# dimalit/ipt

Hardware: AMD Instinct MI355X
Metric: Mpaths/sec at 1024^2, 8-bounce, sample_scenes[0]; achieved HBM GB/s (higher is better)
Workload: dtype f32; 1 GPU; c2: box 1024x1024, 1280 spp, depth_max 8, n_rays 16; width=1024, height=1024, spp=1280, depth_max=8, n_rays=16, tile_rows=0, calls=queued (ipt_render_device_async), one wait, parallelism=tiles1, per_rank=the whole frame's tiles dealt round-robin; 256 x N passes per step (weak)

## Files before the change

ipt_amd/csrc/ipt_kernels.hip:

```cpp
#include <hip/hip_runtime.h>

#include <algorithm>
#include <array>
#include <cmath>
#include <cstdio>
#include <cstdlib>
#include <cstring>
#include <strings.h>
#include <mutex>
#include <string>
#include <thread>
#include <type_traits>
#include <vector>

#include "../../include/ipt_capi.h"
#include "ipt_bvh.h"
#include "ipt_internal.h"
#include "ipt_path.h"
#include "ipt_knobs.h"
#include "ipt_diag.h"

using namespace ipt;

namespace {
// ... 783 lines not shown
        const bool sharded = !(kp.n_shards <= 1 || kp.tile_rows <= 0);
        uint4 r0, r1;
        compact_record(kp, (uint32_t)unit, sharded, r0, r1);
        if (c < kp.total_units) {
            rg[2 * c] = r0;
            rg[2 * c + 1] = r1;
            src[c] = (uint32_t)unit;
        }
    }
}

__global__ void compact_preset_kernel(const unsigned int* __restrict__ blocks, unsigned int nblk,
                                      unsigned long long total_units, unsigned long long* __restrict__ unit_counter,
                                      unsigned long long* __restrict__ ring) {
    if (blockIdx.x != 0 || threadIdx.x != 0) return;
    const unsigned long long n_active = blocks[nblk];
    const unsigned long long start = (total_units - n_active) / kPoolChunk * kPoolChunk;
    *unit_counter = start;
    ring[0] = start;
    ring[1] = n_active;
}

__global__ __launch_bounds__(256) void compact_expand_kernel(const CompactBufs cb, unsigned int nblk,
                                                             unsigned long long total_units) {
    const unsigned long long c = (unsigned long long)blockIdx.x * blockDim.x + threadIdx.x;
    if (c >= total_units || c < total_units - cb.blocks[nblk]) return;
    cb.values[cb.src[c]] = cb.cvalues[c];
}

template <int MAXSUSP, bool COUNT, int LMODE, int GEOM, bool BOXIN, int FIXED>
__global__ __launch_bounds__(block_of(LMODE, GEOM), waves_per_simd(GEOM, LMODE)) void path_kernel(const KParams kp) {
    static_assert(!BOXIN || GEOM == IPT_GEOM_SPHERE_IN_BOX, "BOXIN is the box instances' parameter");
    static_assert(!FIXED || (BOXIN && step_fixed_mode(LMODE)), "FIXED: in-range box instances with a skip-ahead plane");
    static_assert(FIXED >= kFixedPow2 && FIXED <= MAXSUSP, "FIXED = K: K suspended levels");
    constexpr bool kFixed = FIXED != 0;
    constexpr int kK = FIXED > 0 ? FIXED : 0;
    constexpr int kTreeRays = 1 << kK, kTreeMetaShift = kTreeRays > 255 ? 16 : 8;
    constexpr int kRange = GEOM == IPT_GEOM_SPHERE_IN_BOX ? (BOXIN ? kRangeIn : kRangeGeneric) : kRangeRuntime;
    constexpr bool kNearest = box_nearest(GEOM) && kRange != kRangeGeneric;
    constexpr int kBlock = block_of(LMODE, GEOM);
    extern __shared__ float lds[];
    unsigned long long* wslots = reinterpret_cast<unsigned long long*>(lds);
    float* stk = lds + walk_lds_words(LMODE, GEOM);
    constexpr int kFrameStride = frame_stride(LMODE, GEOM);
    float* lfr = stk + MAXSUSP * kStackFields * kBlock;
    LightDev* lights_lds = reinterpret_cast<LightDev*>(lfr + 12 * kFrameStride);
    float* weights_lds = reinterpret_cast<float*>(lights_lds) + kLdsLights * kLightWords;
    float* cdf_lds = weights_lds + (kLdsLights + 1);
    float* gl_lds = reinterpret_cast<float*>(lights_lds) +
                    (LMODE == kLightsLds ? kLdsLights * kLightWords + 2 * (kLdsLights + 1) : 0);
    constexpr bool kGridL = grid_lights(LMODE);
    BvhNode* lnodes_lds = reinterpret_cast<BvhNode*>(gl_lds + global_light_prefix_words(kp.n_lights, kGridL));
    float* cdf_gl = gl_lds + (kGridL ? 0 : kp.n_lights + 1);
    constexpr bool kLaxLds = lax_in_lds(LMODE);
    float4* lax_lds = reinterpret_cast<float4*>(reinterpret_cast<int*>(lnodes_lds) + ((kp.lg_nu * kp.lg_nv + 3) & ~3));
    int* cdf_lo_lds = reinterpret_cast<int*>(cdf_gl + kp.n_lights + 1);
    const int tid = threadIdx.x;
    const int wave = tid >> 6;
    if (tid < 60) lfr[(tid % 12) * kFrameStride + kBlock + tid / 12] = reinterpret_cast<const float*>(kp.wall_frames)[tid];
    if (LMODE == kLightsLds) {
        const float* src = reinterpret_cast<const float*>(kp.lights);
        float* dst = reinterpret_cast<float*>(lights_lds);
        for (int i = tid; i < kp.n_lights * kLightWords; i += kBlock) dst[i] = src[i];
        for (int i = tid; i <= kp.n_lights; i += kBlock) {
            weights_lds[i] = kp.weights[i];
            cdf_lds[i] = kp.cdf[i];
        }
    }
    if (global_lights(LMODE)) {
        const bool int_cdf = kp.cdf_p2;
        for (int i = tid; i <= kp.n_lights; i += kBlock) {
            if (!kGridL) gl_lds[i] = kp.weights[i];
            cdf_gl[i] = int_cdf ? __uint_as_float(cdf_threshold24(kp.cdf[i])) : kp.cdf[i];
        }
        if (kp.cdf_lo)
            for (int i = tid; i < kCdfBuckets; i += kBlock) cdf_lo_lds[i] = kp.cdf_lo[i];
        if (grid_lights(LMODE))
            for (int i = tid; i < kp.lg_nu * kp.lg_nv; i += kBlock) reinterpret_cast<int*>(lnodes_lds)[i] = kp.lgrid[i];
        if (kLaxLds)
            for (int i = tid; i < 3 * kp.n_lights; i += kBlock) lax_lds[i] = kp.lax[i];
        if (LMODE == kLightsGlobal && kp.lnodes_lds) {
            const float4* src = reinterpret_cast<const float4*>(kp.light_nodes);
            float4* dst = reinterpret_cast<float4*>(lnodes_lds);
            for (int i = tid; i < 2 * kp.n_light_nodes; i += kBlock) dst[i] = src[i];
        }
    }
    __syncthreads();
    LightSet<LMODE> LS;
    LS.lds = lights_lds;
    LS.glob = kp.lights;
    LS.wl = global_lights(LMODE) ? gl_lds : weights_lds;
    LS.cl = global_lights(LMODE) ? cdf_gl : cdf_lds;
    LS.wg = kp.weights;
    LS.cg = kp.cdf;
    if (one_light(LMODE)) {
        LS.one = kp.lights[0];
        if (!resumable_geom(GEOM)) {
            vgpr_hold(LS.one.P); vgpr_hold(LS.one.x); vgpr_hold(LS.one.y);
            vgpr_hold(LS.one.n); vgpr_hold(LS.one.inv.c[0]); vgpr_hold(LS.one.inv.c[1]); vgpr_hold(LS.one.inv.c[2]);
        }
        LS.w0 = kp.weights[0];
        LS.c0 = kp.cdf[0];
        LS.c1 = kp.cdf[1];
    }

    auto ltrace = [&](const LightDev& L, vec3 o, vec3 d, vec3* hp, vec3* hn) -> bool {
        if constexpr (LMODE == kLightsOneA10) return light_trace_ax<1, 0, true>(L, o, d, hp, hn);
        else if constexpr (LMODE == kLightsOneA01) return light_trace_ax<0, 1, true>(L, o, d, hp, hn);
        else if constexpr (grid_lights(LMODE) && lattice_a10(LMODE)) return light_trace_ax<1, 0, true>(L, o, d, hp, hn);
        else if constexpr (grid_lights(LMODE)) return light_trace_ax<0, 1, true>(L, o, d, hp, hn);
        else return light_trace<LMODE == kLightsAny>(L, o, d, hp, hn);
    };
    auto lpdf = [&](const LightDev& L, vec3 o, bool h, vec3 hp, vec3 hn) -> float {
        if constexpr (LMODE == kLightsOneA10 || LMODE == kLightsOneA01) return light_pdf_ax<2, true>(L, o, h, hp, hn);
        else if constexpr (grid_lights(LMODE)) return light_pdf_ax<2, true>(L, o, h, hp, hn);
        else return light_pdf(L, o, h, hp, hn);
    };
    auto lsample = [&](const LightDev& L, vec3 o, float a, float b) -> vec3 {
        if constexpr (LMODE == kLightsOneA10) return light_sample_dir_ax<1, 0, true>(L, o, a, b);
        else if constexpr (LMODE == kLightsOneA01) return light_sample_dir_ax<0, 1, true>(L, o, a, b);
        else if constexpr (grid_lights(LMODE) && lattice_a10(LMODE)) return light_sample_dir_ax<1, 0, true>(L, o, a, b);
        else if constexpr (grid_lights(LMODE)) return light_sample_dir_ax<0, 1, true>(L, o, a, b);
        else return light_sample_dir<LMODE == kLightsAny>(L, o, a, b);
    };

    const int lane = tid & 63;
    const uint64_t lanemask_lt = (lane == 0) ? 0ull : (~0ull >> (64 - lane));
    const int nl = one_light(LMODE) ? 1 : kp.n_lights;
    const float w_sdf = kp.weights[nl];
    const unsigned long long per_pass = (unsigned long long)kp.n_cand * (unsigned long long)kp.W;

    __builtin_amdgcn_s_waitcnt(0);

    unsigned long long pool_next = 0, pool_end = 0;

    bool active = true, has_path = false, fresh = false, need_frame = false, need_b = false;
    int pick = -1;
    float u1 = 0.0f, u2 = 0.0f, tr = 0.0f, cs_c = 0.0f, cs_s = 0.0f;
    float pfs = 0.0f, pfc = 0.0f;
    vec3 pto = v3(0, 0, 0);
    bool pfok = false;
    uint32_t unit = 0;
    uint32_t rpass = 0, rpix = 0, k = 0, blk = 0;
    Win8 w;
    vec3 tpos = v3(0, 0, 0);
    int fdepth = -1;
    uint32_t finm = 0;
    constexpr bool kRes = resumable_geom(GEOM);
    constexpr bool kResL = resumable_lights(LMODE, GEOM);
    constexpr bool kBoxHit = !kRes && !kResL && GEOM == IPT_GEOM_SPHERE_IN_BOX && kNearest;
    constexpr bool kFramePf = !(kRes || kResL);
    constexpr bool kSkipAhead = (one_light(LMODE) || grid_lights(LMODE)) && !kResL;
    constexpr bool kPreSkip = kSkipAhead && kFramePf;
    bool tracing = false;
    float xlmix = 0.0f;
    vec3 xro = v3(0, 0, 0), xrd = v3(0, 0, 0), xli_pos = v3(0, 0, 0);
    int xrdepth = 0, xi = 0, xbidx = -1;
    float xli_y = 0.0f;
    bool xis_iter = false, xhas_li = false;
    float xmult = 0.0f, xli_pow = 0.0f, xbest = 0.0f;
    vec3 xtm = v3(0, 0, 0);
    float tres = 0.0f;
    int ti = 0, tdepth = 0, tkind = 0;
    uint32_t c_paths = 0, c_traced = 0, c_surf = 0, c_light = 0, c_exp = 0, c_iter = 0,
             c_lsamp = 0, c_skip = 0, c_sframe = 0, c_ltr = 0, c_drift = 0, c_nodes = 0, c_tests = 0,
             c_lnode = 0, c_ltest = 0;
    IPT_DIAG_STATE

    for (;;) {
        IPT_STAMP_AT(0);
        const bool need = active && !has_path;
        const uint64_t needmask = __ballot(need);
        if (needmask) {
            const int cnt = __popcll(needmask);
            const int rank = __popcll(needmask & lanemask_lt);
            unsigned long long avail = pool_end - pool_next;
            unsigned long long my = 0;
            if ((unsigned long long)cnt > avail) {
                unsigned long long base = 0;
                if (lane == __ffsll((long long)needmask) - 1) {
                    base = atomicAdd(kp.unit_counter, (unsigned long long)kPoolChunk);
                    if (kp.drained && base + kPoolChunk >= kp.total_units)
                        __hip_atomic_store(kp.drained, kp.drain_seq, __ATOMIC_RELAXED, __HIP_MEMORY_SCOPE_SYSTEM);
                }
                base = __shfl(base, __ffsll((long long)needmask) - 1);
                if ((unsigned long long)rank < avail)
                    my = pool_next + rank;
                else
                    my = base + (rank - avail);
                pool_next = base + (cnt - avail);
                pool_end = base + kPoolChunk;
            } else {
                my = pool_next + rank;
                pool_next += cnt;
            }
            if (need) {
                if (my >= kp.total_units) {
                    active = false;
                } else {
                    unit = (uint32_t)my;
                    has_path = true;
                    fresh = true;
                }
            }
        }

        IPT_STAMP_AT(1);
        if (active) { IPT_PHASE(0); }
        auto pop_node = [&]() {
        if (has_path && (kFramePf || !fresh) && !((kRes || kResL) && tracing) && ti >= ((kK > 0 ? kTreeRays : kp.n_rays) >> tdepth)) {
            IPT_PHASE(1);
            const uint32_t m = ~finm & ((1u << tdepth) - 1u);
            const int stop = m ? 31 - (int)__clz(m) : -1;
            constexpr int kLevelWords = kStackFields * kBlock;
            const lds_float* sb = (const lds_float*)(stk + tid);
            auto lvl = [&](int l) { return sb + __umul24((uint32_t)(l < 0 ? 0 : l), (uint32_t)kLevelWords); };
            const lds_float* bs = lvl(stop);
            const float s0 = bs[0 * kBlock], s1 = bs[1 * kBlock], s2 = bs[2 * kBlock];
            const float s3 = bs[3 * kBlock], s4 = bs[4 * kBlock], s5 = bs[5 * kBlock];
            const lds_float* b1 = lvl(tdepth - 1);
            const float r1 = b1[3 * kBlock], m1 = b1[4 * kBlock];
            const lds_float* b2 = lvl(tdepth - 2);
            const float r2 = b2[3 * kBlock], m2 = b2[4 * kBlock];
            uint32_t nr = kK > 0 ? 1u << kK : (uint32_t)kp.n_rays;
            if constexpr (kK == 0) asm volatile("" : "+s"(nr));
            const bool n_pow2 = kFixed || (nr != 0u && (nr & (nr - 1u)) == 0u);
            const uint32_t p2_exp = 96u + (uint32_t)__clz((int)nr);
            float v;
            auto unwind = [&](auto p2) {
                constexpr bool kP2 = decltype(p2)::value;
                const uint32_t sc0 = (p2_exp + (uint32_t)tdepth) << 23;
                auto fin_s = [&](float r, int d, uint32_t sc) {
                    const float q = kP2 ? r * __uint_as_float(sc) : r / (float)(kp.n_rays >> (d < 0 ? 0 : d));
                    return isfinite_(r) ? q : 0.0f;
                };
                v = fin_s(tres, tdepth, sc0);
                const float v1 = fin_s(r1 + (m1 * 1.0f) * v, tdepth - 1, sc0 - (1u << 23));
                v = tdepth - 1 > stop ? v1 : v;
                const float v2 = fin_s(r2 + (m2 * 1.0f) * v, tdepth - 2, sc0 - (2u << 23));
                v = tdepth - 2 > stop ? v2 : v;
                uint32_t sc = sc0 - (3u << 23);
#pragma unroll 1
                for (int l = tdepth - 3; l > stop; --l, sc -= 1u << 23) {
                    const lds_float* b = lvl(l);
                    const float r = b[3 * kBlock] + (b[4 * kBlock] * 1.0f) * v;
                    v = 0.0f;
                    if (isfinite_(r)) v = kP2 ? r * __uint_as_float(sc) : r / (float)(kp.n_rays >> l);
                }
            };
            if constexpr (kFixed)
                unwind(std::true_type{});
            else if (n_pow2)
                unwind(std::true_type{});
            else
                unwind(std::false_type{});
            if (stop >= 0) {
                const int meta = __float_as_int(s5);
                tpos = v3(s0, s1, s2);
                tres = s3 + (s4 * 1.0f) * v;
                tkind = (int)((uint32_t)meta >> (kK > 0 ? kTreeMetaShift : kp.meta_shift));
                ti = (int)__builtin_amdgcn_ubfe((uint32_t)meta, 0u, (uint32_t)(kK > 0 ? kTreeMetaShift : kp.meta_shift));
                need_frame = tkind >= 5 && fdepth != stop;
                tdepth = stop;
                vgpr_hold(tpos);
                vgpr_hold(tdepth);
            } else {
                kp.values[unit] = v >= 0.0f ? v : 0.0f;
                has_path = false;
            }
        }
        };
        if (!kFramePf) pop_node();

        IPT_STAMP_AT(2);
        auto frame_normal = [&]() -> vec3 {
            vec3 nrm;
            if (GEOM == IPT_GEOM_SPHERE_IN_BOX || tkind == 5) {
                nrm = tpos;
            } else {
                const float4 sp = kp.spheres[tkind - 6];
                nrm = tpos - v3(sp.x, sp.y, sp.z);
                if (GEOM == IPT_GEOM_SMALLPT && !((double)sp.w < 100.0)) nrm = -nrm;
            }
            return nrm;
        };
        constexpr bool kFrameInrange = GEOM == IPT_GEOM_SPHERE_IN_BOX;
        const bool fneed = need_frame && has_path && !fresh && !((kRes || kResL) && tracing);
        IPT_STAMP_AT(3);
        const bool iter_lane = has_path && !fresh && !((kRes || kResL) && tracing);
        if constexpr (kRes) {
            pick = -1;
            u1 = u2 = tr = cs_c = cs_s = 0.0f;
        }
        uint32_t gi_a = 0, gi_b = 0;
        bool gcos = false;
        uint32_t pre_w;
        bool pre_ok = false;
        bool pre_ft;
        vec3 lpP = v3(0, 0, 0);
        float lpx = 0.0f, lpy = 0.0f, lpn = 0.0f;
        int lptype = 0;
        auto gathers = [&](bool ran) {
            if constexpr (kRes || kResL) {
                if (ran && gcos) {
                    tr = kp.cos_a[gi_a];
                    float sp, cp;
                    sincosf_small_(two_pi_times_u24(gi_b), &sp, &cp);
                    cs_c = cp;
                    cs_s = sp;
                }
            } else {
                if constexpr (grid_lights(LMODE)) {
                    const int pk = (ran && pick >= 0 && pick < nl) ? pick : 0;
                    const float4 a = kLaxLds ? lax_lds[3 * pk] : kp.lax[3 * pk];
                    lpP = v3(a.x, a.y, kp.lg_pn);
                    lpx = a.z;
                    lpy = a.w;
                    lpn = kp.lg_nn;
                    lptype = 0;
                }
                tr = kp.cos_a[gcos ? gi_a : 0u];
                float sp, cp;
                sincosf_small_(two_pi_times_u24(gi_b), &sp, &cp);
                cs_c = cp;
                cs_s = sp;
            }
        };
        auto prologue = [&]() {
            if ((k >> 2) != blk) {
                w.a0 = w.b0; w.a1 = w.b1; w.a2 = w.b2; w.a3 = w.b3;
                ++blk;
                need_b = true;
            }
            if (need_b) {
                IPT_PHASE(4);
                philox_fill(w.b0, w.b1, w.b2, w.b3, blk + 1, rpass, rpix, kp.key0, kp.key1);
                need_b = false;
            }
            const uint32_t j = kPreSkip ? k - 4u * blk : k & 3u;
            const uint32_t rw = kPreSkip && j >= 4u ? (j & 1u ? w.b1 : w.b0) : sel4(j & 3u, w.a0, w.a1, w.a2, w.a3);
            const float r = u01(rw);
            auto pick_w = [&](uint32_t wd) {
                return (unsigned long long)wd < kp.pk_u0 ? 0 : ((unsigned long long)wd < kp.pk_u1 ? 1 : 2);
            };
            constexpr bool kPickInt = one_light(LMODE);
            auto pick_of = [&](float r) {
                int c = 0;
                if (global_lights(LMODE) && kp.cdf_lo) {
                    c = cdf_lo_lds[(int)(r * 256.0f)];
                    if (kp.cdf_bsearch) {
                        const float f0 = LS.cdf(min(c, nl)), f1 = LS.cdf(min(c + 1, nl)), f2 = LS.cdf(min(c + 2, nl));
                        const int n0 = (c <= nl && !(r < f0)) ? 1 : 0;
                        const int n1 = (c + 1 <= nl && !(r < f1)) ? 1 : 0;
                        const int n2 = (c + 2 <= nl && !(r < f2)) ? 1 : 0;
                        const bool more = n2 != 0;
                        c += n0 + n1 + n2;
                        if (__builtin_expect(__any(more), 0))
                            if (more) while (c <= nl && !(r < LS.cdf(c))) ++c;
                    } else {
                        while (c <= nl && !(r < LS.cdf(c))) ++c;
                    }
                } else if ((global_lights(LMODE) || LMODE == kLightsAny) && kp.cdf_bsearch) {
                    int hi = nl + 1;
                    while (c < hi) {
                        const int mid = (c + hi) >> 1;
                        if (r < LS.cdf(mid)) hi = mid; else c = mid + 1;
                    }
                } else {
                    while (c <= nl && !(r < LS.cdf(c))) ++c;
                }
                return c;
            };
            auto pick_p2w = [&](uint32_t wd) {
                const uint32_t g = wd >> 8;
                const int ce = min((int)(g >> (24 - kp.cdf_p2e)), nl);
                if (kp.cdf_p2 == 2) {
                    return ce < nl ? ce : (g < kp.cdf_end_t ? nl : nl + 1);
                }
                const uint32_t fa = __float_as_uint(LS.cdf(max(ce - 1, 0))), fb = __float_as_uint(LS.cdf(ce));
                int c = (ce >= 1 && g < fa) ? ce - 1 : (g < fb ? ce : ce + 1);
                if (c >= nl) c = g < kp.cdf_end_t ? nl : nl + 1;
                return c;
            };
            constexpr bool kPickIntCdf = global_lights(LMODE);
            auto pick_word = [&](uint32_t wd) {
                if constexpr (kPickInt) return pick_w(wd);
                if constexpr (kPickIntCdf)
                    if (kp.cdf_p2) return pick_p2w(wd);
                return pick_of(u01(wd));
            };
            int c = (kPickInt || kPickIntCdf) ? pick_word(rw) : pick_of(r);
            uint32_t jj = j;
            if constexpr (kSkipAhead) {
                const bool back = (tpos.z - kp.sa_pz) * kp.sa_nz < 0.0f;
                if ((kFixed || kp.sa_on) && c < nl && back && j <= 1u && ti + 1 < ((kK > 0 ? kTreeRays : kp.n_rays) >> tdepth)) {
                    ++ti;
                    if (COUNT) { ++c_iter; ++c_lsamp; ++c_skip; }
                    k += 3;
                    jj = j + 3u;
                    c = pick_word(j == 0u ? w.a3 : w.b0);
                }
            }
            pick = c;
            if (c <= nl) {
                uint32_t r1, r2;
                if constexpr (kPreSkip) {
                    const bool odd = (jj & 1u) != 0u, h0 = jj < 2u, h2 = jj >= 4u;
                    auto sel3 = [&](uint32_t x0, uint32_t x1, uint32_t x2) {
                        const uint32_t t = h0 ? x0 : x1;
                        return h2 ? x2 : t;
                    };
                    const uint32_t e1 = sel3(w.a1, w.a3, w.b1), e2 = sel3(w.a2, w.b0, w.b2);
                    const uint32_t e3 = sel3(w.a3, w.b1, w.b3), e4 = h0 ? w.b0 : w.b2;
                    r1 = odd ? e2 : e1;
                    r2 = odd ? e3 : e2;
                    pre_w = odd ? e4 : e3;
                    pre_ok = jj <= 3u && (kFixed || kp.sa_on);
                    if constexpr (kK > 0 && !COUNT)
                        pre_ft = kPickIntCdf ? (pre_w >> 8) >= kp.cdf_end_t : pick_word(pre_w) > nl;
                } else {
                    const bool hi = kSkipAhead && jj >= 4u;
                    r1 = hi ? w.b1 : sel4(jj & 3u, w.a1, w.a2, w.a3, w.b0);
                    r2 = hi ? w.b2 : sel4(jj & 3u, w.a2, w.a3, w.b0, w.b1);
                }
                u1 = u01(r1);
                u2 = u01(r2);
                if (c == nl) {
                    gi_a = r1 >> 8;
                    gi_b = r2 >> 8;
                    gcos = true;
                }
                k += 3;
            } else {
                k += 1;
            }
        };
        if (iter_lane) {
            IPT_PHASE(3);
            prologue();
        }
        gathers(iter_lane);
        if (fneed) {
            const vec3 nrm = frame_normal();
            IPT_PHASE(5);
            Frame f;
            if (GEOM == IPT_GEOM_SPHERE_IN_BOX) {
                vec3 to;
                float fs = 0.0f, fc = 0.0f;
                if (kFramePf) {
                    if (__builtin_expect(__any(!pfok), 0))
                        if (!pfok) {
                            pto = kFrameInrange ? normalize_inrange_(nrm) : normalize(nrm);
                            frame_sc_lookup(kp.frame_sc, pto, pfs, pfc);
                            keep_alive(pfs);
                            keep_alive(pfc);
                        }
                    to = pto;
                    fs = pfs;
                    fc = pfc;
                    pfok = false;
                } else {
                    to = kFrameInrange ? normalize_inrange_(nrm) : normalize(nrm);
                    frame_sc_lookup(kp.frame_sc, to, fs, fc);
                }
                if (kFrameInrange) {
                    bool ok;
                    f = make_frame_sc_fast(to, fs, fc, ok);
                    if (__builtin_expect(__any(!ok), 0))
                        if (!ok) f = make_frame_sc<kFrameInrange>(to, fs, fc);
                } else {
                    f = make_frame_sc<kFrameInrange>(to, fs, fc);
                }
            } else if (kFrameInrange) {
                f = make_frame<true>(normalize_inrange_(nrm));
            } else {
                const vec3 to = normalize(nrm);
                float fs, fc;
                frame_angle_sc(to, &fs, &fc);
                bool ok;
                f = make_frame_sc_fast(to, fs, fc, ok);
                if (__builtin_expect(__any(!ok), 0))
                    if (!ok) f = make_frame_sc<false>(to, fs, fc);
            }
            float* c = lfr + tid;
            c[0 * kFrameStride] = f.m0.x; c[1 * kFrameStride] = f.m0.y; c[2 * kFrameStride] = f.m0.z;
            c[3 * kFrameStride] = f.m1.x; c[4 * kFrameStride] = f.m1.y; c[5 * kFrameStride] = f.m1.z;
            c[6 * kFrameStride] = f.m2.x; c[7 * kFrameStride] = f.m2.y; c[8 * kFrameStride] = f.m2.z;
            c[9 * kFrameStride] = f.iz.x; c[10 * kFrameStride] = f.iz.y; c[11 * kFrameStride] = f.iz.z;
            need_frame = false;
            fdepth = tdepth;
        }
        if (IPT_PROF && wave == 0) { IPT_PHASE(11); }
        IPT_STAMP_AT(4);
        if (!__ballot(active)) break;
        IPT_STAMP_AT(5);
        const float* frc = lfr + (tkind < 5 ? kBlock + tkind : tid);

        bool have_ray = false, is_iter = false;
        vec3 rd;
        int rdepth;
        if (has_path && fresh) {
            IPT_PHASE(2);
            uint4 r0 = kp.rg[2 * unit], r1 = kp.rg[2 * unit + 1];
            keep_alive(r0);
            keep_alive(r1);
            if (r0.w == 0u) {
                has_path = false;
            } else {
                tpos = kp.cam_pos;
                rd = v3(__uint_as_float(r0.x), __uint_as_float(r0.y), __uint_as_float(r0.z));
                w.a2 = r1.x;
                w.a3 = r1.y;
                rpass = r1.z;
                rpix = r1.w;
                blk = 0;
                need_b = true;
                k = 2;
                rdepth = 0;
                have_ray = true;
                if (COUNT) ++c_paths;
            }
        }
        fresh = false;

        vec3 dir_bf = v3(0, 0, 0);
        constexpr bool kDirBf = one_light(LMODE);
        if constexpr (kDirBf) {
            Frame fm;
            fm.m0 = v3(frc[0 * kFrameStride], frc[1 * kFrameStride], frc[2 * kFrameStride]);
            fm.m1 = v3(frc[3 * kFrameStride], frc[4 * kFrameStride], frc[5 * kFrameStride]);
            fm.m2 = v3(frc[6 * kFrameStride], frc[7 * kFrameStride], frc[8 * kFrameStride]);
            const vec3 cdir = frame_apply(fm, v3(tr * cs_c, tr * cs_s, sqrt_inrange_(u1)));
            const vec3 zero = v3(0, 0, 0);
            if constexpr (LMODE == kLightsOneA10 || LMODE == kLightsOneA01) {
                bool lok;
                const vec3 ldir = LMODE == kLightsOneA10
                                      ? light_sample_dir_ax_ok<1, 0, true>(LS.one, tpos, u1, u2, &lok)
                                      : light_sample_dir_ax_ok<0, 1, true>(LS.one, tpos, u1, u2, &lok);
                const vec3 other = pick == nl ? cdir : zero;
                dir_bf = pick < nl && lok ? ldir : other;
            } else {
                const vec3 ldir = lsample(LS.one, tpos, u1, u2);
                dir_bf = pick < nl ? ldir : (pick == nl ? cdir : zero);
            }
        }
        if (iter_lane) {
            vec3 dir = v3(0, 0, 0);
            if (kDirBf) {
                dir = dir_bf;
                if (COUNT && pick < nl) ++c_lsamp;
            } else if (pick < nl) {
                IPT_PHASE(7);
                if constexpr (grid_lights(LMODE)) {
                    constexpr int XA = lattice_a10(LMODE) ? 1 : 0, YA = 1 - XA;
                    dir = light_sample_dir_axf<XA, YA, true>(lpP, lpx, lpy, lpn, lptype, tpos, u1, u2);
                } else
                dir = lsample(LS.light(pick), tpos, u1, u2);
                if (COUNT) ++c_lsamp;
            } else if (pick == nl) {
                Frame fm;
                fm.m0 = v3(frc[0 * kFrameStride], frc[1 * kFrameStride], frc[2 * kFrameStride]);
                fm.m1 = v3(frc[3 * kFrameStride], frc[4 * kFrameStride], frc[5 * kFrameStride]);
                fm.m2 = v3(frc[6 * kFrameStride], frc[7 * kFrameStride], frc[8 * kFrameStride]);
                dir = frame_apply(fm, v3(tr * cs_c, tr * cs_s, sqrt_inrange_(u1)));
            }
            ++ti;
            if (COUNT) ++c_iter;
            if (is_zero(dir)) {
                if (COUNT) ++c_skip;
            } else {
                rd = dir;
                rdepth = tdepth + 1;
                have_ray = true;
                is_iter = true;
            }
        }
        const vec3 ro = tpos;
        IPT_STAMP_AT(8);
        vec3 box_hitp;
        auto resolve = [&](bool traced, float t, int prim, vec3 o, vec3 d, int depth, bool iter, float mult,
                           bool has_li, float li_y, float li_pow) {
            float cv = 0.0f;
            bool push = false;
            vec3 si_pos = v3(0, 0, 0);
            {
                const bool has_si = prim >= 0;
                if (COUNT && traced) {
                    ++c_traced;
                    c_surf += has_si ? 1u : 0u;
                    c_light += has_li ? 1u : 0u;
                }
                if constexpr (kBoxHit)
                    si_pos = box_hitp;
                else
                    si_pos = o + d * t;
                const vec3 ea = si_pos - o;
                const float x = dot(ea, ea), y = li_y;
                const bool need = has_li && has_si;
                bool lg = x > y * 1.000001907f && y >= 1e-30f;
                const bool tie = need && (!lg && !(x <= y));
                if (__builtin_expect(__any(tie), 0))
                    if (tie) lg = sqrt_(x) > sqrt_(y);
                const bool li_wins = has_li && (!has_si || lg);
                const int nchild = (kK > 0 ? kTreeRays : kp.n_rays) >> depth;
                const float zero = 0.0f;
                const float cv_exp = nchild == 0 ? zero / (float)nchild : 0.0f;
                cv = li_wins ? (isfinite_(li_pow) ? li_pow : 1.0f) : (has_si ? cv_exp : 0.0f);
                cv = traced ? cv : 0.0f;
                push = traced && !li_wins && has_si && nchild != 0;
                if (COUNT && traced && !li_wins && has_si) ++c_exp;
            }
            if (push) {
                IPT_PHASE(10);
                if (iter) {
                    const uint32_t lbit = 1u << tdepth;
                    finm = (finm & ~lbit) | (ti >= ((kK > 0 ? kTreeRays : kp.n_rays) >> tdepth) ? lbit : 0u);
                    lds_float* b = (lds_float*)(stk + tid) + __umul24((uint32_t)tdepth, (uint32_t)(kStackFields * kBlock));
                    b[0 * kBlock] = tpos.x;
                    b[1 * kBlock] = tpos.y;
                    b[2 * kBlock] = tpos.z;
                    b[3 * kBlock] = tres;
                    b[4 * kBlock] = mult;
                    b[5 * kBlock] = __uint_as_float((uint32_t)ti | ((uint32_t)tkind << (kK > 0 ? kTreeMetaShift : kp.meta_shift)));
                }
                tpos = si_pos;
                tkind = prim;
                if (prim >= 5) {
                    need_frame = true;
                    if (COUNT) ++c_sframe;
                }
                tres = 0.0f;
                ti = 0;
                tdepth = depth;
            } else if (iter) {
                tres = tres + (mult * 1.0f) * cv;
            } else {
                kp.values[unit] = cv >= 0.0f ? cv : 0.0f;
                has_path = false;
            }
        };
        if constexpr (kResL) {
            if (have_ray) {
                IPT_PHASE(8);
                if (COUNT) c_ltr += (uint32_t)nl * ((is_iter ? 1u : 0u) + ((rdepth < kp.depth_max) ? 1u : 0u));
                xro = ro;
                xrd = rd;
                xrdepth = rdepth;
// ... 146 lines not shown
                constexpr int XA = lattice_a10(LMODE) ? 1 : 0, YA = 1 - XA;
                const float n_dir = kp.lg_nn * comp<2>(rd);
                const float num = kp.lg_nn * (kp.lg_pn - comp<2>(ro));
                const float t = div_inrange_(num, n_dir);
                lg_ndir = n_dir;
                lg_t = t;
                lg_q = ro + rd * t;
                const float u = (comp<XA>(lg_q) - kp.lg_u0) * kp.lg_icw;
                const float v = (comp<YA>(lg_q) - kp.lg_v0) * kp.lg_ich;
                int cand[4] = {-1, -1, -1, -1};
                const float e = kp.lg_e;
                if (u > -1.0f && u < (float)kp.lg_nu + 1.0f && v > -1.0f && v < (float)kp.lg_nv + 1.0f) {
                    const int i0 = (int)floorf(u - e), i1 = (int)floorf(u + e);
                    const int j0 = (int)floorf(v - e), j1 = (int)floorf(v + e);
                    const int* cells = reinterpret_cast<const int*>(lnodes_lds);
                    auto cell = [&](int i, int j) {
                        const bool in = i >= 0 && i < kp.lg_nu && j >= 0 && j < kp.lg_nv;
                        return in ? cells[i + kp.lg_nu * j] : -1;
                    };
                    cand[0] = cell(i0, j0);
                    cand[1] = i1 != i0 ? cell(i1, j0) : -1;
                    cand[2] = j1 != j0 ? cell(i0, j1) : -1;
                    cand[3] = (i1 != i0 && j1 != j0) ? cell(i1, j1) : -1;
                }
                uint32_t c0 = (uint32_t)cand[0], c1 = (uint32_t)cand[1], c2 = (uint32_t)cand[2], c3 = (uint32_t)cand[3];
                auto cs = [](uint32_t& a, uint32_t& b) { const uint32_t lo = a < b ? a : b; b = a < b ? b : a; a = lo; };
                if (__builtin_expect(__any((c1 & c2 & c3) != 0xffffffffu), 0)) {
                    cs(c0, c1); cs(c2, c3); cs(c0, c2); cs(c1, c3); cs(c1, c2);
                }
                if (c0 != 0xffffffffu) light_step((int)c0);
                if (c1 != 0xffffffffu) light_step((int)c1);
                if (c2 != 0xffffffffu) light_step((int)c2);
                if (c3 != 0xffffffffu) light_step((int)c3);
            } else if (LMODE == kLightsGlobal && kp.n_light_nodes > 0) {
                const vec3 inv = v3(safe_rcp(rd.x), safe_rcp(rd.y), safe_rcp(rd.z));
                auto walk = [&](const BvhNode* __restrict__ lnodes) {
                int i = 0;
                while (i < kp.n_light_nodes) {
                    int leaf = -1;
                    while (i < kp.n_light_nodes) {
                        const BvhNode nd = lnodes[i];
                        if (COUNT) ++c_lnode;
                        const bool enter = bvh_box_entry(nd, ro, inv) != inf_();
                        if (enter && nd.leaf >= 0) {
                            leaf = nd.leaf;
                            i = nd.skip;
                            break;
                        }
                        i = enter ? i + 1 : nd.skip;
                    }
                    if (leaf >= 0) {
                        const int first = leaf & 0xffffff, cnt = leaf >> 24;
                        for (int l = first; l < first + cnt; ++l) light_step(l);
                    }
                }
                };
                if (kp.lnodes_lds)
                    walk(lnodes_lds);
                else
                    walk(kp.light_nodes);
            } else {
                for (int l = 0; l < nl; ++l) light_step(l);
            }
            IPT_STAMP_AT(9);
            float mult = 0.0f;
            if (is_iter) {
                Frame fz;
                fz.iz = v3(frc[9 * kFrameStride], frc[10 * kFrameStride], frc[11 * kFrameStride]);
                const float sdf_val = frame_cosine_value(fz, rd);
                const float mix = lmix + w_sdf * sdf_val;
                mult = div_(sdf_val, mix);
            }
            if (kRes && rdepth < kp.depth_max && (kp.n_nodes > 0 || kp.n_grid > 0)) {
                xrd = rd;
                xis_iter = is_iter;
                xmult = mult;
                xhas_li = has_li;
                {
                    const vec3 eb = li_pos - ro;
                    xli_y = dot(eb, eb);
                }
                xli_pow = li_pow;
                int xp = -1;
                xi = 0;
                xbest = inf_();
                if (GEOM == IPT_GEOM_SPHERES_IN_BOX)
                    xbest = kp.box_inrange ? trace_box_planes_only<true>(ro, rd, &xp)
                                           : trace_box_planes_only<false>(ro, rd, &xp);
                xbidx = -2 - xp;
                if (kp.n_grid > 0) sphere_grid_init(kp, ro, rd, xi, xtm);
                tracing = true;
            } else {
                int prim = -1;
                float t = inf_();
                if (kK > 0 || rdepth < kp.depth_max) {
                    IPT_PHASE(9);
                    t = trace_geometry<COUNT, GEOM, kNearest, kRange>(kp, ro, rd, &prim, &box_hitp, c_nodes, c_tests);
                    IPT_STAMP_AT(10);
                }
                const vec3 eb = li_pos - ro;
                resolve(kK > 0 || rdepth < kp.depth_max, t, prim, ro, rd, rdepth, is_iter, mult, has_li, dot(eb, eb), li_pow);
            }
        }
        IPT_STAMP_AT(11);
        const vec3 xo = xis_iter ? tpos : kp.cam_pos;
        if (kRes && kp.n_grid > 0) {
            if (__ballot(tracing))
                sphere_grid_walk_wave<COUNT>(kp, tracing, xo, xrd, xi, xtm, xbest, xbidx, IPT_GRID_BUDGET,
                                             wslots + (tid & ~63), lane, c_nodes, c_tests IPT_DIAG_ARGS);
            if (tracing && xi < 0) {
                tracing = false;
                if (xbidx >= 0) xbidx = grid_item_index(kp, xbidx);
#if IPT_RAYLOG
                if (!COUNT && kp.raylog) {
                    const unsigned long long k = atomicAdd(kp.raylog_n, 1ull);
                    if (k % kp.raylog_every == 0 && k / kp.raylog_every < kp.raylog_cap) {
                        RayLogRec r;
                        r.o[0] = xo.x; r.o[1] = xo.y; r.o[2] = xo.z; r.t = xbest;
                        r.d[0] = xrd.x; r.d[1] = xrd.y; r.d[2] = xrd.z; r.hit = xbidx;
                        kp.raylog[k / kp.raylog_every] = r;
                    }
                }
#endif
                resolve(true, xbest, xbidx >= 0 ? 6 + xbidx : -2 - xbidx, xo, xrd, xis_iter ? tdepth + 1 : 0, xis_iter,
                        xmult, xhas_li, xli_y, xli_pow);
            }
        } else if (kRes && tracing) {
            IPT_PHASE(9);
            sphere_bvh_walk<COUNT>(kp, xo, xrd, xi, xbest, xbidx, IPT_WALK_BUDGET, c_nodes, c_tests);
            if (xi >= kp.n_nodes) {
                tracing = false;
                resolve(true, xbest, xbidx >= 0 ? 6 + xbidx : -2 - xbidx, xo, xrd, xis_iter ? tdepth + 1 : 0, xis_iter,
                        xmult, xhas_li, xli_y, xli_pow);
            }
        }
        }
        if constexpr (kPreSkip) {
            const bool back = (tpos.z - kp.sa_pz) * kp.sa_nz < 0.0f;
            const bool lpick = (unsigned long long)pre_w < kp.sa_u;
            const bool leaf = kK > 0 && !COUNT && tdepth == kK && (!global_lights(LMODE) || kp.cdf_p2 != 0);
            const bool take = iter_lane && pre_ok && back && ti < ((kK > 0 ? kTreeRays : kp.n_rays) >> tdepth) &&
                              (kK > 0 && !COUNT ? lpick || leaf : lpick);
            ti += take ? 1 : 0;
            k += take ? (kK > 0 && !COUNT ? (pre_ft ? 1u : 3u) : 3u) : 0u;
            if (COUNT) {
                c_iter += take ? 1u : 0u;
                c_lsamp += take ? 1u : 0u;
                c_skip += take ? 1u : 0u;
            }
        }
        if constexpr (kFramePf) {
            pop_node();
            IPT_STAMP_AT(6);
            if constexpr (kFrameInrange) {
                if (need_frame && has_path) {
                    const vec3 to = normalize_inrange_(tpos);
                    const uint32_t u = f2u(to.z), mz = u & 0x7fffffffu;
                    pfok = mz - kFrameTabLo <= kFrameTabSpan;
                    if (pfok) {
                        const float2 e = kp.frame_sc[((mz - kFrameTabLo) << 1) | (u >> 31)];
                        pfs = e.x;
                        pfc = e.y;
                        pto = to;
                    }
                }
            }
            IPT_STAMP_AT(7);
        }
    }

    IPT_DIAG_FLUSH(kp.counters, kNumCounters)
    if (COUNT) {
        atomicAdd(&kp.counters[0], (unsigned long long)c_paths);
        atomicAdd(&kp.counters[1], (unsigned long long)c_traced);
        atomicAdd(&kp.counters[2], (unsigned long long)c_surf);
        atomicAdd(&kp.counters[3], (unsigned long long)c_light);
        atomicAdd(&kp.counters[4], (unsigned long long)c_exp);
        atomicAdd(&kp.counters[5], (unsigned long long)c_iter);
        atomicAdd(&kp.counters[6], (unsigned long long)c_lsamp);
        atomicAdd(&kp.counters[7], (unsigned long long)c_skip);
        atomicAdd(&kp.counters[8], (unsigned long long)c_sframe);
        atomicAdd(&kp.counters[9], (unsigned long long)c_ltr);
        atomicAdd(&kp.counters[10], (unsigned long long)c_drift);
        atomicAdd(&kp.counters[11], (unsigned long long)c_nodes);
        atomicAdd(&kp.counters[12], (unsigned long long)c_tests);
        atomicAdd(&kp.counters[13], (unsigned long long)c_lnode);
        atomicAdd(&kp.counters[14], (unsigned long long)c_ltest);
    }
}

struct PreviewOut {
    uint8_t* kinds;
    float* hits;
};
template <int GEOM>
__device__ __forceinline__ vec3 preview_normal(const KParams& kp, int prim, vec3 pos) {
    if (GEOM == IPT_GEOM_FLOOR) return v3(0.0f, 0.0f, 1.0f);
    if (GEOM == IPT_GEOM_CORNER) return v3(prim == 0 ? 1.0f : 0.0f, prim == 1 ? 1.0f : 0.0f, prim == 2 ? 1.0f : 0.0f);
    if (prim < 5) {
        const float one = prim >= 3 ? 1.0f : -1.0f;
        return v3(prim == 0 || prim == 3 ? one : -0.0f, prim == 1 ? one : -0.0f, prim == 2 || prim == 4 ? one : -0.0f);
    }
    if (GEOM == IPT_GEOM_SPHERE_IN_BOX) return normalize(pos);
    const float4 sp = kp.spheres[prim - 6];
    const vec3 v = normalize(pos - v3(sp.x, sp.y, sp.z));
    if (GEOM == IPT_GEOM_SMALLPT && !((double)sp.w < 100.0)) return -v;
    return v;
}
template <bool FULL, int GEOM>
__global__ __launch_bounds__(256) void preview_kernel(const KParams kp, const PreviewOut po) {
    const unsigned long long unit = (unsigned long long)blockIdx.x * blockDim.x + threadIdx.x;
    const bool in = unit < kp.total_units;
    uint32_t c_nodes = 0, c_tests = 0, c_lnode = 0, c_ltest = 0;
    bool drift = false, valid = false, has_si = false, has_li = false;
    if (in) {
        const bool sharded = !(kp.n_shards <= 1 || kp.tile_rows <= 0);
        const RayGen g = new_path_setup(kp, unit, sharded, kp.cand_rows);
        drift = g.drift;
        valid = g.valid;
        uint8_t kind = 0xff;
        vec3 hpos = v3(0, 0, 0), hnrm = v3(0, 0, 0);
        if (valid) {
            const vec3 o = kp.cam_pos, d = g.rd;
            vec3 li_pos = v3(0, 0, 0);
            auto light_step = [&](int l) {
                vec3 hp, hn;
                const bool h = light_trace<true>(kp.lights[l], o, d, &hp, &hn);
                if (FULL) ++c_ltest;
                if (h && (!has_li || longer(li_pos - o, hp - o))) {
                    has_li = true;
                    li_pos = hp;
                }
            };
            if (kp.n_light_nodes > 0) {
                const vec3 inv = v3(safe_rcp(d.x), safe_rcp(d.y), safe_rcp(d.z));
                int i = 0;
                while (i < kp.n_light_nodes) {
                    const BvhNode nd = kp.light_nodes[i];
                    if (FULL) ++c_lnode;
                    const bool enter = bvh_box_entry(nd, o, inv) != inf_();
                    if (enter && nd.leaf >= 0) {
                        const int first = nd.leaf & 0xffffff, cnt = nd.leaf >> 24;
                        for (int l = first; l < first + cnt; ++l) light_step(l);
                    }
                    i = (enter && nd.leaf < 0) ? i + 1 : nd.skip;
                }
            } else {
                for (int l = 0; l < kp.n_lights; ++l) light_step(l);
            }
            int prim = -1;
            vec3 unused;
            const float t = trace_geometry<FULL, GEOM, false>(kp, o, d, &prim, &unused, c_nodes, c_tests);
            has_si = prim >= 0;
            const vec3 si_pos = o + d * t;
            const bool li_wins = has_li && (!has_si || longer(si_pos - o, li_pos - o));
            float v = li_wins ? 1.0f : 0.0f;
            if (!li_wins && has_si) {
                hnrm = preview_normal<GEOM>(kp, prim, si_pos);
                hpos = si_pos;
                v = div_(dot(hnrm, -d), length(d));
            }
            kp.values[unit] = v >= 0.0f ? v : 0.0f;
            if (li_wins) hpos = li_pos;
            kind = (uint8_t)((li_wins ? 2 : (has_si ? 1 : 0)) | (has_si ? 4 : 0) | (has_li ? 8 : 0));
        }
        if (FULL) {
            if (po.kinds) po.kinds[unit] = kind;
            if (po.hits) {
                float* h = po.hits + 6 * unit;
                h[0] = hpos.x; h[1] = hpos.y; h[2] = hpos.z;
                h[3] = hnrm.x; h[4] = hnrm.y; h[5] = hnrm.z;
            }
        }
    }
    if (FULL && kp.count) {
        const uint32_t nl = valid ? (uint32_t)kp.n_lights : 0u;
        const uint32_t vals[10] = {valid ? 1u : 0u, valid ? 1u : 0u, has_si ? 1u : 0u, has_li ? 1u : 0u, nl,
                                   drift ? 1u : 0u, c_nodes, c_tests, c_lnode, c_ltest};
        const int slot[10] = {0, 1, 2, 3, 9, 10, 11, 12, 13, 14};
        for (int k = 0; k < 10; ++k) {
            const int s = wave_scan_add((int)vals[k]);
            if ((threadIdx.x & 63) == 63 && s) atomicAdd(&kp.counters[slot[k]], (unsigned long long)(uint32_t)s);
        }
    }
}

struct AParams {
    int W, H, spp, n_cand;
    const int* cand_of_row;
    const float* values;
    const uint8_t* codes;
    const uint8_t* flags;
    int tile_rows, n_shards, shard_id;
    float* pixels;
    uint32_t* counters;
    float* sums;
    float* pixel_max;
    unsigned long long* clk;
};
struct AParamsAdapt : AParams {
    const uint8_t* mask;
    float* m2;
};
template <bool ADAPT>
using AParamsOf = std::conditional_t<ADAPT, AParamsAdapt, AParams>;

__device__ __forceinline__ void add_ray(float v, float& p, uint32_t& c, float& s, float& m) {
    p = (p * (float)c + v) / (float)(c + 1u);
    ++c;
    s += v;
    if (p > m) m = p;
// ... 2180 lines not shown
```

ipt_amd/csrc/ipt_knobs.h:

```cpp
#pragma once

#if !defined(IPT_AB_BUILD) &&                                                                    \
    (defined(IPT_BLOCK) || defined(IPT_RES_BLOCK) || defined(IPT_WAVES_PER_SIMD) ||              \
     defined(IPT_RES_WAVES) || defined(IPT_RESL_WAVES) || defined(IPT_GRID_BUDGET) ||            \
     defined(IPT_WALK_BUDGET) || defined(IPT_LWALK_BUDGET) || defined(IPT_BVH_LEAF) ||           \
     defined(IPT_LBVH_LEAF) || defined(IPT_GRID_CELLS_PER_SPHERE) || defined(IPT_C2_ONLY) ||     \
     defined(IPT_C2_LMODE))
#error "an ipt_knobs.h parameter is overridden: A/B builds must define IPT_AB_BUILD"
#endif

#ifndef IPT_BLOCK
#define IPT_BLOCK 256
#endif
#ifndef IPT_RES_BLOCK
#define IPT_RES_BLOCK 64
#endif
#ifndef IPT_WAVES_PER_SIMD
#define IPT_WAVES_PER_SIMD 4
#endif
#ifndef IPT_RES_WAVES
#define IPT_RES_WAVES 4
#endif
#ifndef IPT_RESL_WAVES
#define IPT_RESL_WAVES 3
#endif

#ifndef IPT_GRID_BUDGET
#define IPT_GRID_BUDGET 8
#endif
#ifndef IPT_WALK_BUDGET
#define IPT_WALK_BUDGET 48
#endif
#ifndef IPT_LWALK_BUDGET
#define IPT_LWALK_BUDGET 16
#endif
#ifndef IPT_BVH_LEAF
#define IPT_BVH_LEAF 16
#endif
#ifndef IPT_LBVH_LEAF
#define IPT_LBVH_LEAF 2
#endif
#ifndef IPT_GRID_CELLS_PER_SPHERE
#define IPT_GRID_CELLS_PER_SPHERE 1.5
#endif

#ifndef IPT_C2_ONLY
#define IPT_C2_ONLY 0
#endif
#ifndef IPT_C2_LMODE
#define IPT_C2_LMODE kLightsOneA10
#endif
```

Before: 430.7 Mpaths/s.

## Gate frame construction to alternate iterations and replace wave votes with masks

Adds a frame gate for the sphere-in-box, one-light path. By default (gate mode 1) frame construction and the frame prefetch run only on every other loop iteration, and lanes that need a frame stall on the off iterations. The aim is to batch divergent frame work so more lanes do it together. It also replaces the __ballot/__any votes with precomputed wave masks built from scalar compare intrinsics (uicmp). This may delay some lanes' path progress by an iteration in exchange for better coherence.

```diff
diff --git a/ipt_amd/csrc/ipt_kernels.hip b/ipt_amd/csrc/ipt_kernels.hip
--- a/ipt_amd/csrc/ipt_kernels.hip
+++ b/ipt_amd/csrc/ipt_kernels.hip
@@ -959,6 +959,13 @@
     constexpr bool kFramePf = !(kRes || kResL);
     constexpr bool kSkipAhead = (one_light(LMODE) || grid_lights(LMODE)) && !kResL;
     constexpr bool kPreSkip = kSkipAhead && kFramePf;
+    constexpr int kFrameGate = kFramePf && GEOM == IPT_GEOM_SPHERE_IN_BOX && one_light(LMODE) ? IPT_FRAME_GATE : 0;
+    constexpr bool kGatePf = kFrameGate != 0 && IPT_FRAME_GATE_PF != 0;
+    constexpr bool kMaskVotes = kFramePf && GEOM == IPT_GEOM_SPHERE_IN_BOX;
+    uint64_t active_m = ~0ull;
+    uint32_t pfd = 0xffffffffu;
+    bool fg_run = true;
+    bool fg_any = false;
     bool tracing = false;
     float xlmix = 0.0f;
     vec3 xro = v3(0, 0, 0), xrd = v3(0, 0, 0), xli_pos = v3(0, 0, 0);
@@ -1001,6 +1008,8 @@
                 my = pool_next + rank;
                 pool_next += cnt;
             }
+            if constexpr (kMaskVotes)
+                active_m &= ~(__builtin_amdgcn_uicmpl(my, kp.total_units, 35 ) & needmask);
             if (need) {
                 if (my >= kp.total_units) {
                     active = false;
@@ -1092,9 +1101,15 @@
             return nrm;
         };
         constexpr bool kFrameInrange = GEOM == IPT_GEOM_SPHERE_IN_BOX;
-        const bool fneed = need_frame && has_path && !fresh && !((kRes || kResL) && tracing);
+        bool fneed = need_frame && has_path && !fresh && !((kRes || kResL) && tracing);
+        bool fstall = false;
+        if constexpr (kFrameGate != 0) {
+            fstall = fneed && !fg_run;
+            fneed = fneed && fg_run;
+        }
         IPT_STAMP_AT(3);
-        const bool iter_lane = has_path && !fresh && !((kRes || kResL) && tracing);
+        bool iter_lane = has_path && !fresh && !((kRes || kResL) && tracing);
+        if constexpr (kFrameGate != 0) iter_lane = iter_lane && !fstall;
         if constexpr (kRes) {
             pick = -1;
             u1 = u2 = tr = cs_c = cs_s = 0.0f;
@@ -1255,8 +1270,16 @@
                 vec3 to;
                 float fs = 0.0f, fc = 0.0f;
                 if (kFramePf) {
-                    if (__builtin_expect(__any(!pfok), 0))
-                        if (!pfok) {
+                    bool pf_miss, pf_any;
+                    if constexpr (kMaskVotes) {
+                        pf_miss = pfd > kFrameTabSpan;
+                        pf_any = __builtin_amdgcn_uicmp(pfd, (uint32_t)kFrameTabSpan, 34 ) != 0;
+                    } else {
+                        pf_miss = !pfok;
+                        pf_any = __any(!pfok);
+                    }
+                    if (__builtin_expect(pf_any, 0))
+                        if (pf_miss) {
                             pto = kFrameInrange ? normalize_inrange_(nrm) : normalize(nrm);
                             frame_sc_lookup(kp.frame_sc, pto, pfs, pfc);
                             keep_alive(pfs);
@@ -1266,6 +1289,7 @@
                     fs = pfs;
                     fc = pfc;
                     pfok = false;
+                    if constexpr (kMaskVotes) pfd = 0xffffffffu;
                 } else {
                     to = kFrameInrange ? normalize_inrange_(nrm) : normalize(nrm);
                     frame_sc_lookup(kp.frame_sc, to, fs, fc);
@@ -1299,7 +1323,11 @@
         }
         if (IPT_PROF && wave == 0) { IPT_PHASE(11); }
         IPT_STAMP_AT(4);
-        if (!__ballot(active)) break;
+        if constexpr (kMaskVotes) {
+            if (!active_m) break;
+        } else {
+            if (!__ballot(active)) break;
+        }
         IPT_STAMP_AT(5);
         const float* frc = lfr + (tkind < 5 ? kBlock + tkind : tid);
 
@@ -1752,11 +1780,19 @@
         if constexpr (kFramePf) {
             pop_node();
             IPT_STAMP_AT(6);
+            if constexpr (kFrameGate == 1) fg_run = !fg_run;
+            if constexpr (kFrameGate == 2) {
+                const bool waited = !fg_run && fg_any;
+                const uint64_t nm = __ballot(need_frame && has_path);
+                fg_any = nm != 0;
+                fg_run = __popcll(nm) >= IPT_FRAME_GATE_T || waited;
+            }
             if constexpr (kFrameInrange) {
-                if (need_frame && has_path) {
+                if (need_frame && has_path && (!kGatePf || fg_run)) {
                     const vec3 to = normalize_inrange_(tpos);
                     const uint32_t u = f2u(to.z), mz = u & 0x7fffffffu;
                     pfok = mz - kFrameTabLo <= kFrameTabSpan;
+                    if constexpr (kMaskVotes) pfd = mz - kFrameTabLo;
                     if (pfok) {
                         const float2 e = kp.frame_sc[((mz - kFrameTabLo) << 1) | (u >> 31)];
                         pfs = e.x;
diff --git a/ipt_amd/csrc/ipt_knobs.h b/ipt_amd/csrc/ipt_knobs.h
--- a/ipt_amd/csrc/ipt_knobs.h
+++ b/ipt_amd/csrc/ipt_knobs.h
@@ -5,7 +5,8 @@
      defined(IPT_RES_WAVES) || defined(IPT_RESL_WAVES) || defined(IPT_GRID_BUDGET) ||            \
      defined(IPT_WALK_BUDGET) || defined(IPT_LWALK_BUDGET) || defined(IPT_BVH_LEAF) ||           \
      defined(IPT_LBVH_LEAF) || defined(IPT_GRID_CELLS_PER_SPHERE) || defined(IPT_C2_ONLY) ||     \
-     defined(IPT_C2_LMODE))
+     defined(IPT_C2_LMODE) || defined(IPT_FRAME_GATE) || defined(IPT_FRAME_GATE_T) ||            \
+     defined(IPT_FRAME_GATE_PF))
 #error "an ipt_knobs.h parameter is overridden: A/B builds must define IPT_AB_BUILD"
 #endif
 
@@ -44,6 +45,16 @@
 #define IPT_GRID_CELLS_PER_SPHERE 1.5
 #endif
 
+#ifndef IPT_FRAME_GATE
+#define IPT_FRAME_GATE 1
+#endif
+#ifndef IPT_FRAME_GATE_T
+#define IPT_FRAME_GATE_T 8
+#endif
+#ifndef IPT_FRAME_GATE_PF
+#define IPT_FRAME_GATE_PF 1
+#endif
+
 #ifndef IPT_C2_ONLY
 #define IPT_C2_ONLY 0
 #endif
```

Result: no change. 432.5 Mpaths/s (median of 6 runs) (+0.4%).
